# AmandineBtto/NeRAF

Hardware: AMD Instinct MI355X
Metric: field-samples/sec (rays + RIR STFT bins) (higher is better)
Workload: dtype f16; 1 GPU; RAF FurnishedRoom joint training step (BASELINE configs[2]): 4096 rays + 2048 RIR slices x 513 bins per GPU; radiance + grid refresh + ResNet3D + NAcF + STFT loss, backward, GradScaler + fused Adam...; rays_per_gpu=4096, slices_per_gpu=2048, global_rays=4096, global_slices=2048, parallelism=dp1, distinct_resident_batches=16, deterministic=True

## Files before the change

include/neraf_hip.h:

```cpp
#ifndef NERAF_HIP_H
#define NERAF_HIP_H

#include <stddef.h>
#include <stdint.h>

#ifdef __cplusplus
extern "C" {
#endif

typedef struct neraf_ctx neraf_ctx;
typedef void* neraf_stream_t;

enum {
  NERAF_OK = 0,
  NERAF_EINVAL = -1,
  NERAF_EHIP = -2,
  NERAF_ENOGPU = -3,
  NERAF_ESTATE = -4
};

#define NERAF_ABI_VERSION 1

int neraf_abi_version(void);
int neraf_ctx_create(neraf_ctx** out, int device);
void neraf_ctx_destroy(neraf_ctx* ctx);
const char* neraf_last_error(neraf_ctx* ctx);

int neraf_graph_stats(neraf_ctx* ctx, int* captures, int* launches);
int neraf_prof_enable(neraf_ctx* ctx, int on);
int neraf_prof_summary(neraf_ctx* ctx, int kernel_id, double* total_ms, int* launches, double* work);
int neraf_prof_summary_ex(neraf_ctx* ctx, int kernel_id, double* total_ms, int* launches, double* work, double* exec_work);
int neraf_prof_event_overhead(neraf_ctx* ctx, void* scratch_word, neraf_stream_t stream, double* ms);
const char* neraf_prof_kernel_name(int kernel_id);

int neraf_gemm_f16(neraf_ctx* ctx, const void* A, int lda, const void* B, int ldb, int M, int N, int K,
                   int Mpad, int Npad, float alpha, const float* bias, int act,
                   void* C16, int ldc16, void* C16T, int ldc16t, float* C32, int ldc32,
                   neraf_stream_t stream);

int neraf_gemm_f16_grouped(neraf_ctx* ctx, int ngroups, const void* const* A, const void* const* B, const int* M, const int* N,
                           float* const* C32, const int* ldc32, int lda, int ldb, int K, float alpha, const float* alpha_dev,
                           int c32_beta, void* splitk_ws, size_t splitk_bytes, neraf_stream_t stream);

int neraf_gemm_f16_stream(neraf_ctx* ctx, const void* A, int lda, const void* B, int ldb, int M, int N, int K, int Mpad, int Npad,
                          float alpha, const float* bias, const void* add16, int ldadd, void* C16, int ldc16, void* C16T,
                          int ldc16t, float* C32, int ldc32, float* colsum, float* colsumsq, int stat_rep, int stat_stride,
                          int stat_det, int body, int max_workgroups, neraf_stream_t stream);

int neraf_gemm_bf16(neraf_ctx* ctx, const void* A, int lda, const void* B, int ldb, int M, int N, int K,
                    int Mpad, int Npad, float alpha, const float* bias, int act,
                    void* C16, int ldc16, void* C16T, int ldc16t, float* C32, int ldc32,
                    neraf_stream_t stream);
int neraf_gemm_bf16_tn(neraf_ctx* ctx, const void* A, const void* B, int M, int N, int K, float* C32, void* splitk_ws,
                       size_t splitk_bytes, neraf_stream_t stream);

typedef struct neraf_nacf_desc {
  int n_feat;
  int n_query;
  int W;
  int C;
  int F;
  int dense_l0;
} neraf_nacf_desc;

size_t neraf_nacf_packed_bytes(const neraf_nacf_desc* d);
size_t neraf_nacf_workspace_bytes(const neraf_nacf_desc* d, int B, int training);

int neraf_nacf_pack_weights(neraf_ctx* ctx, const neraf_nacf_desc* d, const float* const* weights,
                            void* packed, neraf_stream_t stream);

int neraf_nacf_encode_queries(neraf_ctx* ctx, const neraf_nacf_desc* d, const int64_t* time_query,
                              const double* mic_pose, const double* source_pose, const double* rot,
                              const float* aabb_host, int max_len, int B, void* workspace, int training,
                              neraf_stream_t stream);
int neraf_nacf_encode_queries_ex(neraf_ctx* ctx, const neraf_nacf_desc* d, const int64_t* time_query,
                                 const double* mic_pose, const double* source_pose, const double* rot, int pose_rows,
                                 const float* aabb_host, int max_len, int B, void* workspace, int training,
                                 neraf_stream_t stream);

int neraf_nacf_fwd(neraf_ctx* ctx, const neraf_nacf_desc* d, const void* packed, const float* const* weights,
                   const float* feat, int B, float* out, void* workspace, int training, neraf_stream_t stream);

int neraf_nacf_fwd_dense(neraf_ctx* ctx, const neraf_nacf_desc* d, const void* packed, const float* h, int B,
                         float* out, void* workspace, int training, neraf_stream_t stream);

int neraf_nacf_bwd(neraf_ctx* ctx, const neraf_nacf_desc* d, const void* packed, const float* const* weights,
                   const float* feat, int B, const float* out, const float* dout, float* const* grads,
                   float* dfeat, void* workspace, neraf_stream_t stream);

int neraf_nacf_bwd_dense(neraf_ctx* ctx, const neraf_nacf_desc* d, const void* packed, int B, const float* out,
                         const float* dout, float* const* grads, float* dh, void* workspace,
                         neraf_stream_t stream);

#define NERAF_STFT_SUMS_FLOATS (4 + 4 * 256)
int neraf_stft_loss_fwd(neraf_ctx* ctx, const float* pred, const float* gt, size_t n, int loss_type,
                        float* sums, float* losses, neraf_stream_t stream);
int neraf_stft_loss_sums(neraf_ctx* ctx, const float* pred, const float* gt, size_t n, int loss_type,
                         float* sums, neraf_stream_t stream);
int neraf_stft_loss_finalize(neraf_ctx* ctx, const float* sums, size_t n_total, const float* weights, float* losses,
                             neraf_stream_t stream);
// ... 200 lines not shown
```

neraf_amd/_lib.py:

```python
from __future__ import annotations

import ctypes as C
import os
from typing import Dict, Optional

_HERE = os.path.dirname(os.path.abspath(__file__))
LIB_PATH = os.environ.get("NERAF_HIP_LIB") or os.path.join(_HERE, "libneraf_hip.so")

_lib: Optional[C.CDLL] = None
_ctxs: Dict[int, C.c_void_p] = {}

c_fpp = C.POINTER(C.c_void_p)


class GridDesc(C.Structure):
    _fields_ = [("n_levels", C.c_int), ("base_res", C.c_int), ("max_res", C.c_int), ("log2_hashmap_size", C.c_int),
                ("n_features", C.c_int)]


class ResnetDesc(C.Structure):
    _fields_ = [("grid_size", C.c_int), ("in_channels", C.c_int), ("n_features", C.c_int)]


class NacfDesc(C.Structure):
    _fields_ = [("n_feat", C.c_int), ("n_query", C.c_int), ("W", C.c_int), ("C", C.c_int), ("F", C.c_int),
                ("dense_l0", C.c_int)]


SIGNATURES = {
    "neraf_abi_version": (C.c_int, []),
    "neraf_ctx_create": (C.c_int, [C.POINTER(C.c_void_p), C.c_int]),
    "neraf_ctx_destroy": (None, [C.c_void_p]),
    "neraf_last_error": (C.c_char_p, [C.c_void_p]),
    "neraf_gemm_f16": (C.c_int, [C.c_void_p, C.c_void_p, C.c_int, C.c_void_p, C.c_int, C.c_int, C.c_int, C.c_int,
                                 C.c_int, C.c_int, C.c_float, C.c_void_p, C.c_int, C.c_void_p, C.c_int, C.c_void_p,
                                 C.c_int, C.c_void_p, C.c_int, C.c_void_p]),
    "neraf_gemm_f16_grouped": (C.c_int, [C.c_void_p, C.c_int, c_fpp, c_fpp, C.POINTER(C.c_int), C.POINTER(C.c_int), c_fpp,
                                         C.POINTER(C.c_int), C.c_int, C.c_int, C.c_int, C.c_float, C.c_void_p, C.c_int, C.c_void_p, C.c_size_t,
                                         C.c_void_p]),
    "neraf_gemm_f16_stream": (C.c_int, [C.c_void_p, C.c_void_p, C.c_int, C.c_void_p, C.c_int, C.c_int, C.c_int, C.c_int, C.c_int, C.c_int,
                                        C.c_float, C.c_void_p, C.c_void_p, C.c_int, C.c_void_p, C.c_int, C.c_void_p, C.c_int, C.c_void_p,
                                        C.c_int, C.c_void_p, C.c_void_p, C.c_int, C.c_int, C.c_int, C.c_int, C.c_int, C.c_void_p]),
    "neraf_gemm_bf16": (C.c_int, [C.c_void_p, C.c_void_p, C.c_int, C.c_void_p, C.c_int, C.c_int, C.c_int, C.c_int,
                                  C.c_int, C.c_int, C.c_float, C.c_void_p, C.c_int, C.c_void_p, C.c_int, C.c_void_p,
                                  C.c_int, C.c_void_p, C.c_int, C.c_void_p]),
    "neraf_gemm_bf16_tn": (C.c_int, [C.c_void_p, C.c_void_p, C.c_void_p, C.c_int, C.c_int, C.c_int, C.c_void_p, C.c_void_p, C.c_size_t,
                                     C.c_void_p]),
    "neraf_fused_adam_chunk": (C.c_int, []),
    "neraf_grads_nonfinite": (C.c_int, [C.c_void_p, C.c_void_p, C.c_void_p, C.c_void_p, C.c_void_p, C.c_int, C.c_void_p, C.c_void_p, C.c_int,
                                        C.c_int, C.c_void_p]),
    "neraf_fused_adam": (C.c_int, [C.c_void_p, C.c_void_p, C.c_void_p, C.c_void_p, C.c_void_p, C.c_int, C.c_void_p, C.c_int, C.c_int,
                                   C.c_double, C.c_double, C.c_double, C.c_void_p, C.c_void_p, C.c_void_p, C.c_void_p]),
    "neraf_fused_adam_dual": (C.c_int, [C.c_void_p, C.c_void_p, C.c_void_p, C.c_void_p, C.c_void_p, C.c_int, C.c_void_p, C.c_int, C.c_int,
                                        C.c_double, C.c_double, C.c_double, C.c_void_p, C.c_void_p, C.c_void_p, C.c_void_p, C.c_void_p,
                                        C.c_void_p, C.c_void_p, C.c_int, C.c_void_p, C.c_int, C.c_void_p]),
    "neraf_nacf_packed_bytes": (C.c_size_t, [C.POINTER(NacfDesc)]),
    "neraf_nacf_workspace_bytes": (C.c_size_t, [C.POINTER(NacfDesc), C.c_int, C.c_int]),
    "neraf_nacf_pack_weights": (C.c_int, [C.c_void_p, C.POINTER(NacfDesc), c_fpp, C.c_void_p, C.c_void_p]),
    "neraf_nacf_encode_queries": (C.c_int, [C.c_void_p, C.POINTER(NacfDesc), C.c_void_p, C.c_void_p, C.c_void_p,
                                            C.c_void_p, C.POINTER(C.c_float), C.c_int, C.c_int, C.c_void_p, C.c_int,
                                            C.c_void_p]),
    "neraf_nacf_encode_queries_ex": (C.c_int, [C.c_void_p, C.POINTER(NacfDesc), C.c_void_p, C.c_void_p, C.c_void_p,
                                               C.c_void_p, C.c_int, C.POINTER(C.c_float), C.c_int, C.c_int, C.c_void_p, C.c_int,
                                               C.c_void_p]),
    "neraf_nacf_fwd": (C.c_int, [C.c_void_p, C.POINTER(NacfDesc), C.c_void_p, c_fpp, C.c_void_p, C.c_int, C.c_void_p,
                                 C.c_void_p, C.c_int, C.c_void_p]),
    "neraf_nacf_fwd_dense": (C.c_int, [C.c_void_p, C.POINTER(NacfDesc), C.c_void_p, C.c_void_p, C.c_int, C.c_void_p,
                                       C.c_void_p, C.c_int, C.c_void_p]),
    "neraf_nacf_bwd": (C.c_int, [C.c_void_p, C.POINTER(NacfDesc), C.c_void_p, c_fpp, C.c_void_p, C.c_int, C.c_void_p,
                                 C.c_void_p, c_fpp, C.c_void_p, C.c_void_p, C.c_void_p]),
    "neraf_nacf_bwd_dense": (C.c_int, [C.c_void_p, C.POINTER(NacfDesc), C.c_void_p, C.c_int, C.c_void_p, C.c_void_p,
                                       c_fpp, C.c_void_p, C.c_void_p, C.c_void_p]),
    "neraf_stft_loss_fwd": (C.c_int, [C.c_void_p, C.c_void_p, C.c_void_p, C.c_size_t, C.c_int, C.c_void_p, C.c_void_p,
                                      C.c_void_p]),
    "neraf_stft_loss_sums": (C.c_int, [C.c_void_p, C.c_void_p, C.c_void_p, C.c_size_t, C.c_int, C.c_void_p, C.c_void_p]),
    "neraf_stft_loss_finalize": (C.c_int, [C.c_void_p, C.c_void_p, C.c_size_t, C.c_void_p, C.c_void_p, C.c_void_p]),
    "neraf_stft_loss_bwd": (C.c_int, [C.c_void_p, C.c_void_p, C.c_void_p, C.c_size_t, C.c_size_t, C.c_int, C.c_void_p,
                                      C.c_void_p, C.c_void_p, C.c_void_p, C.c_float, C.c_void_p, C.c_void_p]),
    "neraf_prof_event_overhead": (C.c_int, [C.c_void_p, C.c_void_p, C.c_void_p, C.POINTER(C.c_double)]),
    "neraf_graph_stats": (C.c_int, [C.c_void_p, C.POINTER(C.c_int), C.POINTER(C.c_int)]),
    "neraf_prof_enable": (C.c_int, [C.c_void_p, C.c_int]),
    "neraf_prof_summary": (C.c_int, [C.c_void_p, C.c_int, C.POINTER(C.c_double), C.POINTER(C.c_int), C.POINTER(C.c_double)]),
    "neraf_prof_summary_ex": (C.c_int, [C.c_void_p, C.c_int, C.POINTER(C.c_double), C.POINTER(C.c_int), C.POINTER(C.c_double),
                                        C.POINTER(C.c_double)]),
    "neraf_prof_kernel_name": (C.c_char_p, [C.c_int]),
    "neraf_grid_layout": (C.c_int, [C.POINTER(GridDesc), C.POINTER(C.c_float), C.POINTER(C.c_int), C.POINTER(C.c_uint32),
                                    C.POINTER(C.c_uint32)]),
    "neraf_hash_encode": (C.c_int, [C.c_void_p, C.POINTER(GridDesc), C.c_void_p, C.c_void_p, C.c_longlong, C.c_void_p, C.c_void_p]),
    "neraf_sample_uniform": (C.c_int, [C.c_void_p, C.c_int, C.c_int, C.c_float, C.c_float, C.c_void_p, C.c_uint64, C.c_void_p,
                                       C.c_void_p, C.c_void_p]),
    "neraf_proposal_density": (C.c_int, [C.c_void_p, C.POINTER(GridDesc), C.c_void_p, C.c_void_p, C.c_void_p, C.c_void_p,
                                         C.c_void_p, C.c_int, C.c_int, C.c_float, C.c_int, C.c_void_p, C.c_void_p]),
    "neraf_proposal_density_ex": (C.c_int, [C.c_void_p, C.POINTER(GridDesc), C.c_void_p, C.c_void_p, C.c_void_p, C.c_void_p,
                                            C.c_void_p, C.c_int64, C.c_int, C.c_int, C.c_float, C.c_int, C.c_void_p, C.c_void_p]),
    "neraf_pdf_resample_ex": (C.c_int, [C.c_void_p, C.c_void_p, C.c_void_p, C.c_void_p, C.c_int64, C.c_int, C.c_int, C.c_float,
# ... 163 lines not shown
```

neraf_amd/csrc/common.h:

```cpp
#pragma once
#include <hip/hip_runtime.h>
#include <stdint.h>
#include <stdio.h>
#include <new>
#include <string>
#include <vector>

#include "../../include/neraf_hip.h"

typedef _Float16 half_t;
typedef _Float16 half8 __attribute__((ext_vector_type(8)));
typedef _Float16 half4 __attribute__((ext_vector_type(4)));
typedef _Float16 half2v __attribute__((ext_vector_type(2)));
typedef __bf16 bf16_t;
typedef __bf16 bf16x8 __attribute__((ext_vector_type(8)));
typedef __bf16 bf16x4 __attribute__((ext_vector_type(4)));
typedef float f32x4 __attribute__((ext_vector_type(4)));
typedef float f32x16 __attribute__((ext_vector_type(16)));

enum { PROF_GEMM128 = 0, PROF_GEMM64 = 1, PROF_PROP_DENSITY = 2, PROF_FIELD_QUERY = 3, PROF_CONV = 4, PROF_PROP_BWD = 5, PROF_FIELD_BWD = 6,
       PROF_FIELD_SCATTER = 7, PROF_GEMM_WIDE = 8, PROF_WGRAD = 9, PROF_GEMM64_BF16 = 10, PROF_GEMM12864 = 11,
       PROF_CONV64_BF16 = 12, PROF_CONV12864 = 13, PROF_CONV128 = 14, PROF_CONV_STEM = 15, PROF_NUM_KERNELS = 16 };

struct ProfRec { hipEvent_t a, b; int kid; double work; double exec; };
// ... 124 lines not shown
  size_t blocks = (words + 256 - 1) / 256;
  if (blocks > 4096) blocks = 4096;
  hipLaunchKernelGGL(neraf_zero3_kernel, dim3((unsigned)blocks), dim3(256), 0, st, (unsigned*)p0, w0, (unsigned*)p1, w1, (unsigned*)p2, w2);
}

static inline bool neraf_deterministic() {
  static const bool d = [] { const char* e = getenv("NERAF_DETERMINISTIC"); return e && atoi(e) != 0; }();
  return d;
}

static inline int round_up(int x, int m) { return (x + m - 1) / m * m; }
static inline size_t round_up_sz(size_t x, size_t m) { return (x + m - 1) / m * m; }

enum { ACT_NONE = 0, ACT_LEAKY = 1, ACT_TANH10 = 2, ACT_RELU = 3 };

struct ConvGeom {
  int loader;
  int din, dout, stride, pad, ksize, cin;
  int tflip;
  int tstride;
  int tclass;
  const half_t* zero_page;
};

struct GemmParams {
  const half_t* A; int lda;
  const half_t* B; int ldb;
  int M, N, K;
  int Mpad, Npad;
  float alpha;
  const float* alpha_dev;
  const float* bias;
  int act;
  const half_t* lmask; int ldmask;
  float mask_slope;
  const half_t* add16; int ldadd;
  half_t* C16; int ldc16;
  half_t* C16T; int ldc16t;
  float* C32; int ldc32;
  int c32_beta;
  float* colsum;
  float* colsumsq;
  int stat_rep, stat_stride;
  int stat_det;
  const half_t* bnb_x; int ldbnb;
  const half_t* bnb_mask;
  const float* bnb_fin; int bnb_cpad;
  ConvGeom conv;
  float* splitk_ws; size_t splitk_ws_bytes;
  int tile_n;
  double alg_flops;
  int bf16;
  int stream_body, stream_max_wg;
  int ngroups;
  struct Group { const half_t* A; const half_t* B; float* C32; int M, N, ldc32; int tile_begin; } grp[6];
};
constexpr int kMaxGemmGroups = 6;

int launch_gemm_f16(neraf_ctx* ctx, const GemmParams& p, hipStream_t stream);

struct WgradItem {
  const void* dy;
  const void* x;
  float* out;
  int cout, cin, cin_real, ksize, stride, pad, din, dout;
  int K;
  int alpha_idx;
};
int launch_wgrad_grouped(neraf_ctx* ctx, const WgradItem* items, int n, const half_t* zero_page, float* slab_ws, size_t slab_bytes,
                         const float* alpha_dev, hipStream_t stream, bool bf16 = false);

constexpr int kAmaxRep = 32, kAmaxStride = 64;
```

neraf_amd/csrc/gemm_f16.hip:

```cpp
#include "common.h"
#include <stdlib.h>
#include <type_traits>

namespace {

constexpr int BK = 64;

__device__ __forceinline__ float act_apply(float v, int act) {
  if (act == ACT_LEAKY) return v > 0.f ? v : 0.1f * v;
  if (act == ACT_TANH10) return 10.f * tanhf(v);
  if (act == ACT_RELU) return v > 0.f ? v : 0.f;
  return v;
}

template <bool BF> struct ET;
template <> struct ET<false> {
  typedef _Float16 s; typedef half8 v8; typedef half4 v4;
  static __device__ __forceinline__ f32x4 mfma(v8 a, v8 b, f32x4 c) { return __builtin_amdgcn_mfma_f32_16x16x32_f16(a, b, c, 0, 0, 0); }
};
template <> struct ET<true> {
  typedef __bf16 s; typedef bf16x8 v8; typedef bf16x4 v4;
  static __device__ __forceinline__ f32x4 mfma(v8 a, v8 b, f32x4 c) { return __builtin_amdgcn_mfma_f32_16x16x32_bf16(a, b, c, 0, 0, 0); }
};

// ... 679 lines not shown
  __shared__ float tile2[32][33];
  if (p.bnb_x) {
#pragma unroll
    for (int r = 0; r < 4; ++r) tile2[row][c4 + r] = v[r] * (((float)xv[r] - mu[r]) * rsqrtf(var[r] + 1e-5f));
  }
  if (p.C16) {
    E4 h;
#pragma unroll
    for (int r = 0; r < 4; ++r) h[r] = (E)v[r];
    *reinterpret_cast<E4*>(reinterpret_cast<E*>(p.C16) + (size_t)m * p.ldc16 + n) = h;
  }
  if (C32 && m < M) {
    float* dst = C32 + (size_t)m * ldc32 + n;
    if (n + 3 < N && (reinterpret_cast<size_t>(dst) & 15) == 0) {
      f32x4 o = v;
      if (p.c32_beta) o += *reinterpret_cast<const f32x4*>(dst);
      *reinterpret_cast<f32x4*>(dst) = o;
    } else {
#pragma unroll
      for (int r = 0; r < 4; ++r) if (n + r < N) dst[r] = v[r] + (p.c32_beta ? dst[r] : 0.f);
    }
  }
  __syncthreads();
  const int tx = t & 31, ty = t >> 5;
  if (p.C16T) {
#pragma unroll
    for (int i = 0; i < 4; ++i) {
      const int nn = n0 + ty + i * 8, mm = m0 + tx;
      reinterpret_cast<E*>(p.C16T)[(size_t)nn * p.ldc16t + mm] = (E)tile[tx][ty + i * 8];
    }
  }
  if ((p.colsum || p.colsumsq) && ty < 2) {
    float cs = 0.f;
    if (ty == 0) {
#pragma unroll 8
      for (int i = 0; i < 32; ++i) cs += tile[i][tx];
    } else if (p.bnb_x) {
#pragma unroll 8
      for (int i = 0; i < 32; ++i) cs += tile2[i][tx];
    } else {
#pragma unroll 8
      for (int i = 0; i < 32; ++i) { const float x = tile[i][tx]; cs += x * x; }
    }
    float* dst = ty == 0 ? p.colsum : p.colsumsq;
    if (p.stat_det) {
      if (dst) dst[(size_t)blockIdx.y * p.stat_stride + n0 + tx] = cs;
    } else {
      const int rep = p.stat_rep > 1 ? (blockIdx.y & (p.stat_rep - 1)) * p.stat_stride : 0;
      if (dst) atomicAdd(dst + rep + n0 + tx, cs);
    }
  }
}

static void gemm_manifest(neraf_ctx* ctx, const GemmParams& p, int loader, int splits, int bm, int bn, double flops, bool wide = false, bool stream = false) {
  double out_elems = (double)p.M * p.N;
  double rA = loader == 0 ? (double)p.M * p.K * 2.0 : (double)p.conv.din * p.conv.din * p.conv.din * p.conv.cin * 2.0;
  double rB = (double)p.N * p.K * 2.0;
  const int ng = p.ngroups > 1 ? p.ngroups : 1;
  if (ng > 1) {
    out_elems = rA = rB = 0.0;
    for (int g = 0; g < ng; ++g) { out_elems += (double)p.grp[g].M * p.grp[g].N; rA += (double)p.grp[g].M * p.K * 2.0; rB += (double)p.grp[g].N * p.K * 2.0; }
  }
  const double epi_r = out_elems * 2.0 * ((p.add16 ? 1 : 0) + (p.lmask ? 1 : 0) + (p.bnb_mask ? 1 : 0) + (p.bnb_x ? 1 : 0));
  const double epi_w = out_elems * (2.0 * ((p.C16 ? 1 : 0) + (p.C16T ? 1 : 0)) + (p.C32 ? 4.0 : 0.0));
  const double slabs = (double)splits * ng * p.Mpad * p.Npad * 4.0;
  char nm[96];
  if (ng > 1)
    snprintf(nm, sizeof(nm), "gemm_f16_nt_pipe_kernel<%d, %d | plain, %d groups, %.0f results K=%d%s", bm, bn, ng, out_elems, p.K, splits > 1 ? " splitK" : "");
  else
    snprintf(nm, sizeof(nm), "%s<%d, %d | %s M=%d N=%d K=%d%s",
             stream ? "gemm_f16_nt_stream_kernel" : (wide ? "gemm_f16_nt_wide_kernel" : "gemm_f16_nt_pipe_kernel"), bm, bn,
             loader == 0 ? "plain" : (p.conv.tflip ? "dgrad" : "conv"), p.M, p.N, p.K, splits > 1 ? " splitK" : "");
  if (splits > 1) {
    neraf_node(ctx, nm, flops, rA + rB, slabs);
    neraf_node(ctx, "splitk_reduce_kernel | K-split slabs -> result", 0.0, slabs + epi_r, epi_w);
  } else {
    neraf_node(ctx, nm, flops, rA + rB + epi_r, epi_w);
  }
}

template <int BM, int BN, int NST, int LOADER, int KS, bool BF, bool TC = false, int NW = 4, bool GRP = false>
int launch_pipe(neraf_ctx* ctx, const GemmParams& p_in, int splits, hipStream_t stream) {
  using PT = PipeTile<BM, BN, NST>;
  GemmParams p = p_in;
  if ((p.ngroups > 1) != GRP) return neraf_fail(ctx, NERAF_EINVAL, "gemm: grouped launches take the grouped instantiation");
  int grp_tiles = 0;
  if (GRP) {
    for (int g = 0; g < p.ngroups; ++g) {
      p.grp[g].tile_begin = grp_tiles;
      grp_tiles += ((p.grp[g].M + BM - 1) / BM) * ((p.grp[g].N + BN - 1) / BN);
    }
  }
  static bool attr_set = false;
  if (!attr_set) {
    NERAF_HIP_CHECK(ctx, hipFuncSetAttribute(reinterpret_cast<const void*>(&gemm_f16_nt_pipe_kernel<BM, BN, NST, LOADER, KS, BF, TC, NW, GRP>),
                                             hipFuncAttributeMaxDynamicSharedMemorySize, PT::LDS_BYTES));
    attr_set = true;
  }
  const int ng = p.ngroups > 1 ? p.ngroups : 1;
  const int ntiles = GRP ? grp_tiles : (p.Mpad / BM) * (p.Npad / BN);
  double flops = 2.0 * p.M * p.N * p.K;
  if (ng > 1) { flops = 0.0; for (int g = 0; g < ng; ++g) flops += 2.0 * p.grp[g].M * p.grp[g].N * p.K; }
  const double exec_flops = (LOADER != 0 && p.conv.tstride > 1) ? (p.alg_flops > 0.0 ? p.alg_flops : flops) : flops;
  if (p.alg_flops > 0.0) flops = p.alg_flops;
  constexpr int kid = LOADER == 2 ? PROF_CONV_STEM
                      : LOADER == 1 ? (BM * BN == 128 * 128 ? PROF_CONV128 : (BM == 128 ? PROF_CONV12864 : (BF ? PROF_CONV64_BF16 : PROF_CONV)))
                                    : (BM * BN == 128 * 128 ? PROF_GEMM128 : (BM == 128 ? PROF_GEMM12864 : (BF ? PROF_GEMM64_BF16 : PROF_GEMM64)));
  ProfScope prof(ctx, stream, kid, flops, exec_flops);
  hipLaunchKernelGGL((gemm_f16_nt_pipe_kernel<BM, BN, NST, LOADER, KS, BF, TC, NW, GRP>), dim3(ntiles * splits), dim3(NW * 64), PT::LDS_BYTES,
                     stream, p, splits);
  NERAF_HIP_CHECK(ctx, hipGetLastError());
  if (ctx && ctx->manifest) gemm_manifest(ctx, p, LOADER, splits, BM, BN, flops);
  if (splits > 1) {
    hipLaunchKernelGGL(splitk_reduce_kernel<BF>, dim3(p.Npad / 32, p.Mpad / 32, ng), dim3(256), 0, stream, p, splits);
    NERAF_HIP_CHECK(ctx, hipGetLastError());
  }
  return NERAF_OK;
}


template <int BM, int BN, int NST, bool BF>
int launch_wide(neraf_ctx* ctx, const GemmParams& p, int splits, hipStream_t stream) {
  using T = Tile<BM, BN, 4>;
  constexpr int LDS_BYTES = (NST * T::STAGE_BYTES > T::NWAVES * T::EPI_BYTES_WAVE) ? NST * T::STAGE_BYTES : T::NWAVES * T::EPI_BYTES_WAVE;
// ... 154 lines not shown
          red[(wave * 2 + 1) * NW + col] = y;
        }
      }
    __syncthreads();
    if (tid < 2 * NW) {
      const int which = tid / NW, col = tid - which * NW;
      float v = 0.f;
#pragma unroll
      for (int w = 0; w < 8; ++w) v += red[(w * 2 + which) * NW + col];
      float* dst = which ? p.colsumsq : p.colsum;
      if (dst) {
        if (p.stat_det) dst[(size_t)((2 * rg * R) >> 5) * p.stat_stride + n_w0 + col] = v;
        else atomicAdd(dst + (p.stat_rep > 1 ? (rg & (p.stat_rep - 1)) * p.stat_stride : 0) + n_w0 + col, v);
      }
    }
  }
}

static bool stream_qualifies(const GemmParams& p) {
  const bool nk = (p.N == 64 || p.N == 128 || p.N == 256) && (p.K == 64 || p.K == 128 || p.K == 256) && p.N * p.K <= 16384;
  return nk && p.Npad == p.N && p.conv.loader == 0 && p.ngroups <= 1 && !p.bf16 && (p.Mpad % kStreamRows) == 0 && p.C16 &&
         !p.bias && !p.act && !p.lmask && !p.C16T && !p.C32 && !p.alpha_dev && !p.bnb_x && !p.bnb_mask &&
         (!p.add16 || (p.ldadd % 4) == 0);
}

template <int N, int K>
int launch_stream_nk(neraf_ctx* ctx, const GemmParams& p, hipStream_t stream) {
  const int nblocks = p.Mpad / kStreamRows;
  constexpr int CS = stream_slices(N);
  int nrg = (ctx ? ctx->num_cus : 256) / CS;
  if (p.stream_max_wg > 0 && nrg > p.stream_max_wg / CS) nrg = p.stream_max_wg / CS;
  if (nrg > (nblocks + 1) / 2) nrg = (nblocks + 1) / 2;
  if (nrg < 1) nrg = 1;
  const int grid = nrg * CS;
  const double flops = p.alg_flops > 0.0 ? p.alg_flops : 2.0 * p.M * p.N * p.K;
  ProfScope prof(ctx, stream, N == 64 ? PROF_GEMM12864 : PROF_GEMM_WIDE, flops, 2.0 * p.M * p.N * p.K);
  if (p.colsum || p.colsumsq) hipLaunchKernelGGL((gemm_f16_nt_stream_kernel<N, K, true>), dim3(grid), dim3(512), 0, stream, p, nblocks, nrg);
  else hipLaunchKernelGGL((gemm_f16_nt_stream_kernel<N, K, false>), dim3(grid), dim3(512), 0, stream, p, nblocks, nrg);
  NERAF_HIP_CHECK(ctx, hipGetLastError());
  if (ctx && ctx->manifest) gemm_manifest(ctx, p, 0, 1, N, K, flops, false, true);
  return NERAF_OK;
}

int launch_stream(neraf_ctx* ctx, const GemmParams& p, hipStream_t stream) {
  switch (p.N * 1000 + p.K) {
    case 64064: return launch_stream_nk<64, 64>(ctx, p, stream);
    case 64128: return launch_stream_nk<64, 128>(ctx, p, stream);
    case 64256: return launch_stream_nk<64, 256>(ctx, p, stream);
    case 128064: return launch_stream_nk<128, 64>(ctx, p, stream);
    case 128128: return launch_stream_nk<128, 128>(ctx, p, stream);
    case 256064: return launch_stream_nk<256, 64>(ctx, p, stream);
  }
  return neraf_fail(ctx, NERAF_EINVAL, "gemm: shape outside the streaming body's");
}

struct WgDesc {
  const void* dy; const void* x; float* out;
  unsigned long long slab_off;
  int block_begin; int K;
  unsigned short cout, cin, cin_real, taps, din, tiles_n, splits;
  unsigned char dl, stride, ksize, loader; signed char pad; unsigned char mh, ai, r2, r3, r4;
};
static_assert(sizeof(WgDesc) == 64, "descriptor table must fit the 4 KiB kernel-argument segment");
constexpr int kMaxWg = 56;
struct WgTable { int n; int total_blocks; const half_t* zero_page; const float* alpha_dev; float* slab; int order; WgDesc d[kMaxWg]; };

__device__ __forceinline__ int wg_find(const WgTable& t, int bid) {
  int lo = 0, hi = t.n - 1;
  while (lo < hi) { const int mid = (lo + hi + 1) >> 1; if (t.d[mid].block_begin <= bid) lo = mid; else hi = mid - 1; }
  return lo;
}

__device__ __forceinline__ size_t wg_out_index(const WgDesc& d, int m, int n) {
  const int tap = n / d.cin, c = n - tap * d.cin;
  return ((size_t)m * d.cin_real + c) * d.taps + tap;
}

template <bool BF> struct TrRead;
template <> struct TrRead<true> {
  static __device__ __forceinline__ bf16x4 rd(const char* p) {
    return __builtin_amdgcn_ds_read_tr16_b64_v4bf16((__attribute__((address_space(3))) bf16x4*)p);
  }
};
template <> struct TrRead<false> {
  typedef __fp16 fp16x4 __attribute__((ext_vector_type(4)));
  static __device__ __forceinline__ half4 rd(const char* p) {
    const fp16x4 v = __builtin_amdgcn_ds_read_tr16_b64_v4f16((__attribute__((address_space(3))) fp16x4*)p);
    return __builtin_bit_cast(half4, v);
  }
};

template <int NST, bool BF>
__global__ __launch_bounds__(256) void wgrad_grouped_tn_kernel(WgTable t) {
  using E = typename ET<BF>::s; using E4 = typename ET<BF>::v4; using E8 = typename ET<BF>::v8;
  constexpr int BM = 64, BN = 64;
  constexpr int STAGE_BYTES = (BM + BN) * 128;
  extern __shared__ __attribute__((aligned(16))) char smem[];
  const int tid = threadIdx.x;
  const int lane = tid & 63;
  const int wave = __builtin_amdgcn_readfirstlane(tid >> 6);
  const int wm = wave >> 1, wn = wave & 1;
  const int gi = wg_find(t, blockIdx.x);
  const WgDesc& D = t.d[gi];
  int bid = blockIdx.x - D.block_begin;
  const int splits = D.splits, tiles_n = D.tiles_n, tiles_m = D.cout / BM;
  const int split = bid % splits;
// ... 367 lines not shown
    *reinterpret_cast<f32x4*>(slab + (size_t)(m_base + row) * Npad + n_base + col) = v;
  }
}

struct WgRedTable { int n; const float* alpha_dev; const float* slab; int tile_begin[kMaxWg + 1]; unsigned char item[kMaxWg]; };

__device__ __forceinline__ int wg_red_cb(const WgDesc& D) { return D.taps == 1 ? (D.cin < 256 ? D.cin : 256) : (D.taps > 32 ? D.cin : (D.cin < 128 ? D.cin : 128)); }

__global__ __launch_bounds__(256) void wgrad_grouped_reduce_kernel(WgTable t, WgRedTable r) {
  __shared__ float blk[3584];
  int lo = 0, hi = r.n - 1;
  const int bid = blockIdx.x;
  while (lo < hi) { const int mid = (lo + hi + 1) >> 1; if (r.tile_begin[mid] <= bid) lo = mid; else hi = mid - 1; }
  const WgDesc& D = t.d[r.item[lo]];
  const int tile = bid - r.tile_begin[lo];
  const int taps = D.taps, cin = D.cin, CB = wg_red_cb(D), cbs = cin / CB;
  const int m = tile / cbs, ci0 = (tile - m * cbs) * CB;
  const int Npad = D.tiles_n * 64;
  const size_t slab = (size_t)D.cout * Npad;
  const float* src = r.slab + D.slab_off + (size_t)m * Npad + ci0;
  const int splits = D.splits, pitch = taps + 1, q4 = CB >> 2, total4 = q4 * taps;
  for (int e = threadIdx.x; e < total4; e += 256) {
    const int tap = e / q4, c = (e - tap * q4) * 4;
    const float* p = src + tap * cin + c;
    f32x4 v = f32x4{0.f, 0.f, 0.f, 0.f};
    int s2 = 0;
    for (; s2 + 8 <= splits; s2 += 8) {
      f32x4 a[8];
#pragma unroll
      for (int u = 0; u < 8; ++u) a[u] = *reinterpret_cast<const f32x4*>(p + (size_t)(s2 + u) * slab);
#pragma unroll
      for (int u = 0; u < 8; ++u) v += a[u];
    }
    for (; s2 < splits; ++s2) v += *reinterpret_cast<const f32x4*>(p + (size_t)s2 * slab);
#pragma unroll
    for (int k = 0; k < 4; ++k) blk[taps == 1 ? c + k : (c + k) * pitch + tap] = v[k];
  }
  __syncthreads();
  const float alpha = r.alpha_dev ? r.alpha_dev[D.ai] : 1.f;
  const int creal = (D.cin_real - ci0) < CB ? (D.cin_real - ci0) : CB;
  float* dst = D.out + ((size_t)m * D.cin_real + ci0) * taps;
  for (int j = threadIdx.x; j < creal * taps; j += 256) {
    const int c = j / taps, tap = j - c * taps;
    dst[j] = blk[taps == 1 ? c : c * pitch + tap] * alpha;
  }
}

static const int kWide = [] { const char* e = getenv("NERAF_GEMM_WIDE"); return e ? atoi(e) : 1; }();
static const int kSplitMinK = [] { const char* e = getenv("NERAF_SPLIT_MIN_K"); return e ? atoi(e) : 32; }();

static bool conv_waves8() { static const bool v = [] { const char* e = getenv("NERAF_CONV_WAVES"); return e && atoi(e) == 8; }(); return v; }

constexpr int kStreamMinM = 32768;

template <int LOADER, int KS, bool BF>
int dispatch_tile(neraf_ctx* ctx, const GemmParams& p_in, hipStream_t stream) {
  GemmParams p = p_in;
  const int cus = ctx ? ctx->num_cus : 256;
  static const int kTclass = [] { const char* e = getenv("NERAF_DGRAD_TCLASS"); return e ? atoi(e) : 1; }();
  p.conv.tclass = 0;
  if (LOADER == 1 && kTclass && p.conv.tstride == 2 && p.conv.tflip && (p.conv.dout & 1) == 0 && p.ngroups <= 1 &&
      p.Mpad == p.conv.dout * p.conv.dout * p.conv.dout && (p.Mpad % 512) == 0 && (p.Npad % 64) == 0 && !p.lmask && !p.C16T && !p.C32 &&
      !p.colsum && !p.colsumsq) {
    p.conv.tclass = 1;
    if constexpr (LOADER == 1) { if (conv_waves8()) return launch_pipe<64, 64, 4, LOADER, KS, BF, true, 8>(ctx, p, 1, stream); }
    return launch_pipe<64, 64, 4, LOADER, KS, BF, LOADER == 1>(ctx, p, 1, stream);
  }
  if (p.stream_body == 1 && !(LOADER == 0 && !BF && stream_qualifies(p)))
    return neraf_fail(ctx, NERAF_EINVAL, "gemm: shape or epilogue outside the streaming body's");
  if constexpr (LOADER == 0 && !BF) {
    const bool det_stats = p.stat_det && (p.colsum || p.colsumsq);
    if (p.stream_body != 2 && stream_qualifies(p) && (p.stream_body == 1 || (p.Mpad >= kStreamMinM && !det_stats)))
      return launch_stream(ctx, p, stream);
  }
  const int nk = p.K / BK;
  int bm = 128, bn = 128;
  const bool can128 = (p.Mpad % 128) == 0 && (p.Npad % 128) == 0;
  static const int kTile64 = [] { const char* e = getenv("NERAF_CONV_TILE64"); return e ? atoi(e) : 1; }();
  if (p.tile_n == 64 && (p.Mpad % 128) == 0 && !(kTile64 && LOADER == 1)) { bm = 128; bn = 64; }
  else if (!can128 || (p.Mpad / 128) * (p.Npad / 128) < cus) { bm = 64; bn = 64; }
  const int ng = p.ngroups > 1 ? p.ngroups : 1;
  int ntiles = (p.Mpad / bm) * (p.Npad / bn);
  bool uniform = true;
  if (ng > 1) {
    bm = 64; bn = 64; ntiles = 0;
    for (int g = 0; g < ng; ++g) {
      ntiles += (round_up(p.grp[g].M, 64) / 64) * (round_up(p.grp[g].N, 64) / 64);
      uniform = uniform && round_up(p.grp[g].M, 64) == p.Mpad && round_up(p.grp[g].N, 64) == p.Npad;
    }
  }
  int splits = 1;
  static const int kOversub = [] { const char* e = getenv("NERAF_SPLIT_OVERSUB"); const int v = e ? atoi(e) : 2; return v < 1 ? 1 : (v > 4 ? 4 : v); }();
  if (p.splitk_ws && uniform && ntiles * 2 <= cus && nk >= kSplitMinK) {
    splits = ((LOADER != 0 && ntiles >= 64) ? kOversub : 1) * cus / ntiles;
    if (splits > nk / 4) splits = nk / 4;
    if (splits > 128) splits = 128;
    while (splits >= 2 && (size_t)splits * ng * p.Mpad * p.Npad * 4 > p.splitk_ws_bytes) splits >>= 1;
    if (splits < 2) splits = 1;
  }
  if (LOADER == 0 && ng == 1 && kWide && (p.Mpad % 256) == 0) {
    if ((p.Npad % 160) == 0 && (p.Mpad / 256) * (p.Npad / 160) * 4 >= cus * 3) return launch_wide<256, 160, 3, BF>(ctx, p, 1, stream);
    if ((p.Npad % 128) == 0 && (p.Mpad / 256) * (p.Npad / 128) >= cus) return launch_wide<256, 128, 3, BF>(ctx, p, 1, stream);
  }
  if (LOADER == 0 && ng == 1 && kWide && bm == 128 && bn == 128 && splits == 1 && ntiles < 2 * cus)
    return launch_wide<128, 128, 3, BF>(ctx, p, 1, stream);
  static const int kTile32 = [] { const char* e = getenv("NERAF_TILE32"); return e ? atoi(e) : 128; }();
  if constexpr (LOADER == 0) {
    if (ng > 1) {
      if (kTile32 && splits == 1 && ntiles <= kTile32) return launch_pipe<32, 32, 4, LOADER, KS, BF, false, 4, true>(ctx, p, 1, stream);
      return launch_pipe<64, 64, 4, LOADER, KS, BF, false, 4, true>(ctx, p, splits, stream);
    }
    if (kTile32 && splits == 1 && bm == 64 && bn == 64 && ntiles <= kTile32 && !p.C16T)
      return launch_pipe<32, 32, 4, LOADER, KS, BF>(ctx, p, 1, stream);
  }
  if (bm == 128 && bn == 128) return launch_pipe<128, 128, 2, LOADER, KS, BF>(ctx, p, splits, stream);
  if (bm == 128 && bn == 64) return launch_pipe<128, 64, 3, LOADER, KS, BF>(ctx, p, splits, stream);
  if constexpr (LOADER == 1) { if (conv_waves8()) return launch_pipe<64, 64, 4, LOADER, KS, BF, false, 8>(ctx, p, splits, stream); }
  return launch_pipe<64, 64, 4, LOADER, KS, BF>(ctx, p, splits, stream);
}

}

int launch_wgrad_grouped(neraf_ctx* ctx, const WgradItem* items, int n, const half_t* zero_page, float* slab_ws, size_t slab_bytes,
                         const float* alpha_dev, hipStream_t stream, bool bf16) {
  if (n <= 0 || n > kMaxWg || !items || !zero_page) return neraf_fail(ctx, NERAF_EINVAL, "wgrad_grouped: bad arguments");
  static const int nst = [] { const char* e = getenv("NERAF_WGRAD_NST"); const int v = e ? atoi(e) : 3; return v < 2 ? 2 : (v > 4 ? 4 : v); }();
// ... 136 lines not shown
      if (p.conv.ksize == 1) return p.bf16 ? dispatch_tile<1, 1, true>(ctx, p, stream) : dispatch_tile<1, 1, false>(ctx, p, stream);
      return neraf_fail(ctx, NERAF_EINVAL, "conv loader 1: ksize must be 1 or 3");
    case 2:
      if (p.conv.cin != 8 || p.conv.ksize != 5 || !p.conv.zero_page || p.bf16) return neraf_fail(ctx, NERAF_EINVAL, "conv loader 2: cin 8, ksize 5, fp16");
      return dispatch_tile<2, 5, false>(ctx, p, stream);
  }
  return neraf_fail(ctx, NERAF_EINVAL, "gemm: unknown loader");
}

extern "C" int neraf_gemm_f16(neraf_ctx* ctx, const void* A, int lda, const void* B, int ldb, int M, int N, int K,
                              int Mpad, int Npad, float alpha, const float* bias, int act, void* C16, int ldc16,
                              void* C16T, int ldc16t, float* C32, int ldc32, neraf_stream_t stream) {
  GemmParams p{};
  p.A = (const half_t*)A; p.lda = lda; p.B = (const half_t*)B; p.ldb = ldb;
  p.M = M; p.N = N; p.K = K; p.Mpad = Mpad; p.Npad = Npad; p.alpha = alpha; p.bias = bias; p.act = act;
  p.C16 = (half_t*)C16; p.ldc16 = ldc16; p.C16T = (half_t*)C16T; p.ldc16t = ldc16t; p.C32 = C32; p.ldc32 = ldc32;
  return launch_gemm_f16(ctx, p, (hipStream_t)stream);
}

extern "C" int neraf_gemm_f16_grouped(neraf_ctx* ctx, int ngroups, const void* const* A, const void* const* B, const int* M, const int* N,
                                      float* const* C32, const int* ldc32, int lda, int ldb, int K, float alpha, const float* alpha_dev,
                                      int c32_beta, void* splitk_ws, size_t splitk_bytes, neraf_stream_t stream) {
  if (ngroups < 1 || ngroups > kMaxGemmGroups || !A || !B || !M || !N || !C32 || !ldc32)
    return neraf_fail(ctx, NERAF_EINVAL, "gemm_f16_grouped: 1 to 6 groups");
  GemmParams p{};
  p.lda = lda; p.ldb = ldb; p.K = K; p.alpha = alpha; p.alpha_dev = alpha_dev; p.c32_beta = c32_beta;
  p.splitk_ws = (float*)splitk_ws; p.splitk_ws_bytes = splitk_ws ? splitk_bytes : 0;
  for (int g = 0; g < ngroups; ++g) {
    if (M[g] <= 0 || N[g] <= 0) return neraf_fail(ctx, NERAF_EINVAL, "gemm_f16_grouped: M and N must be positive");
    GemmParams::Group& G = p.grp[g];
    G.A = (const half_t*)A[g]; G.B = (const half_t*)B[g]; G.C32 = C32[g]; G.M = M[g]; G.N = N[g]; G.ldc32 = ldc32[g];
    if (!G.A || !G.B || !G.C32) return neraf_fail(ctx, NERAF_EINVAL, "gemm_f16_grouped: null operand or result");
  }
  p.ngroups = ngroups;
  return launch_gemm_f16(ctx, p, (hipStream_t)stream);
}

extern "C" int neraf_gemm_f16_stream(neraf_ctx* ctx, const void* A, int lda, const void* B, int ldb, int M, int N, int K, int Mpad, int Npad,
                                     float alpha, const float* bias, const void* add16, int ldadd, void* C16, int ldc16, void* C16T,
                                     int ldc16t, float* C32, int ldc32, float* colsum, float* colsumsq, int stat_rep, int stat_stride,
                                     int stat_det, int body, int max_workgroups, neraf_stream_t stream) {
  if (body < 0 || body > 2 || max_workgroups < 0) return neraf_fail(ctx, NERAF_EINVAL, "gemm_f16_stream: body 0..2, max_workgroups >= 0");
  GemmParams p{};
  p.A = (const half_t*)A; p.lda = lda; p.B = (const half_t*)B; p.ldb = ldb;
  p.M = M; p.N = N; p.K = K; p.Mpad = Mpad; p.Npad = Npad; p.alpha = alpha; p.bias = bias;
  p.add16 = (const half_t*)add16; p.ldadd = ldadd;
  p.C16 = (half_t*)C16; p.ldc16 = ldc16; p.C16T = (half_t*)C16T; p.ldc16t = ldc16t; p.C32 = C32; p.ldc32 = ldc32;
  p.colsum = colsum; p.colsumsq = colsumsq; p.stat_rep = stat_rep; p.stat_stride = stat_stride; p.stat_det = stat_det;
  p.tile_n = N == 64 ? 64 : 0;
  p.stream_body = body; p.stream_max_wg = max_workgroups;
  return launch_gemm_f16(ctx, p, (hipStream_t)stream);
}

extern "C" int neraf_gemm_bf16(neraf_ctx* ctx, const void* A, int lda, const void* B, int ldb, int M, int N, int K,
                               int Mpad, int Npad, float alpha, const float* bias, int act, void* C16, int ldc16,
                               void* C16T, int ldc16t, float* C32, int ldc32, neraf_stream_t stream) {
  GemmParams p{};
  p.bf16 = 1;
  p.A = (const half_t*)A; p.lda = lda; p.B = (const half_t*)B; p.ldb = ldb;
  p.M = M; p.N = N; p.K = K; p.Mpad = Mpad; p.Npad = Npad; p.alpha = alpha; p.bias = bias; p.act = act;
  p.C16 = (half_t*)C16; p.ldc16 = ldc16; p.C16T = (half_t*)C16T; p.ldc16t = ldc16t; p.C32 = C32; p.ldc32 = ldc32;
  return launch_gemm_f16(ctx, p, (hipStream_t)stream);
}

extern "C" int neraf_gemm_bf16_tn(neraf_ctx* ctx, const void* A, const void* B, int M, int N, int K, float* C32, void* splitk_ws,
                                  size_t splitk_bytes, neraf_stream_t stream) {
  if (!A || !B || !C32 || M <= 0 || N <= 0 || K <= 0 || (M % 64) || (N % 64) || (K % 64) || !splitk_ws || splitk_bytes < 256)
    return neraf_fail(ctx, NERAF_EINVAL, "gemm_bf16_tn: M, N, K multiples of 64; scratch required");
  WgradItem it{};
  it.dy = A; it.x = B; it.out = C32;
  it.cout = M; it.cin = N; it.cin_real = N; it.ksize = 1; it.stride = 1; it.pad = 0; it.din = 1; it.dout = 1; it.K = K;
  return launch_wgrad_grouped(ctx, &it, 1, (const half_t*)splitk_ws, (float*)((char*)splitk_ws + 256), splitk_bytes - 256, nullptr,
                              (hipStream_t)stream, true);
}
```

Baseline: 268.5 million field-samples/s.

## Add LDS-resident halo kernel for 3x3x3 64-channel conv3d and its dgrad

```diff
diff --git a/include/neraf_hip.h b/include/neraf_hip.h
--- a/include/neraf_hip.h
+++ b/include/neraf_hip.h
@@ -46,6 +46,10 @@
                           float alpha, const float* bias, const void* add16, int ldadd, void* C16, int ldc16, void* C16T,
                           int ldc16t, float* C32, int ldc32, float* colsum, float* colsumsq, int stat_rep, int stat_stride,
                           int stat_det, int body, int max_workgroups, neraf_stream_t stream);
+
+int neraf_conv3d_f16_body(neraf_ctx* ctx, const void* x, const void* w, const void* zero_page, int edge_in, int edge_out, int cin,
+                          int cout, int ksize, int stride, int pad, int transposed, float alpha, void* C16, float* colsum,
+                          float* colsumsq, int stat_rep, int stat_stride, int stat_det, int body, neraf_stream_t stream);
 
 int neraf_gemm_bf16(neraf_ctx* ctx, const void* A, int lda, const void* B, int ldb, int M, int N, int K,
                     int Mpad, int Npad, float alpha, const float* bias, int act,
diff --git a/neraf_amd/_lib.py b/neraf_amd/_lib.py
--- a/neraf_amd/_lib.py
+++ b/neraf_amd/_lib.py
@@ -41,6 +41,9 @@
     "neraf_gemm_f16_stream": (C.c_int, [C.c_void_p, C.c_void_p, C.c_int, C.c_void_p, C.c_int, C.c_int, C.c_int, C.c_int, C.c_int, C.c_int,
                                         C.c_float, C.c_void_p, C.c_void_p, C.c_int, C.c_void_p, C.c_int, C.c_void_p, C.c_int, C.c_void_p,
                                         C.c_int, C.c_void_p, C.c_void_p, C.c_int, C.c_int, C.c_int, C.c_int, C.c_int, C.c_void_p]),
+    "neraf_conv3d_f16_body": (C.c_int, [C.c_void_p, C.c_void_p, C.c_void_p, C.c_void_p, C.c_int, C.c_int, C.c_int, C.c_int, C.c_int, C.c_int,
+                                        C.c_int, C.c_int, C.c_float, C.c_void_p, C.c_void_p, C.c_void_p, C.c_int, C.c_int, C.c_int, C.c_int,
+                                        C.c_void_p]),
     "neraf_gemm_bf16": (C.c_int, [C.c_void_p, C.c_void_p, C.c_int, C.c_void_p, C.c_int, C.c_int, C.c_int, C.c_int,
                                   C.c_int, C.c_int, C.c_float, C.c_void_p, C.c_int, C.c_void_p, C.c_int, C.c_void_p,
                                   C.c_int, C.c_void_p, C.c_int, C.c_void_p]),
diff --git a/neraf_amd/csrc/common.h b/neraf_amd/csrc/common.h
--- a/neraf_amd/csrc/common.h
+++ b/neraf_amd/csrc/common.h
@@ -200,6 +200,7 @@
   double alg_flops;
   int bf16;
   int stream_body, stream_max_wg;
+  int conv_body;
   int ngroups;
   struct Group { const half_t* A; const half_t* B; float* C32; int M, N, ldc32; int tile_begin; } grp[6];
 };
diff --git a/neraf_amd/csrc/gemm_f16.hip b/neraf_amd/csrc/gemm_f16.hip
--- a/neraf_amd/csrc/gemm_f16.hip
+++ b/neraf_amd/csrc/gemm_f16.hip
@@ -755,7 +755,8 @@
   }
 }
 
-static void gemm_manifest(neraf_ctx* ctx, const GemmParams& p, int loader, int splits, int bm, int bn, double flops, bool wide = false, bool stream = false) {
+static void gemm_manifest(neraf_ctx* ctx, const GemmParams& p, int loader, int splits, int bm, int bn, double flops, bool wide = false, bool stream = false,
+                          bool resident = false) {
   double out_elems = (double)p.M * p.N;
   double rA = loader == 0 ? (double)p.M * p.K * 2.0 : (double)p.conv.din * p.conv.din * p.conv.din * p.conv.cin * 2.0;
   double rB = (double)p.N * p.K * 2.0;
@@ -772,7 +773,7 @@
     snprintf(nm, sizeof(nm), "gemm_f16_nt_pipe_kernel<%d, %d | plain, %d groups, %.0f results K=%d%s", bm, bn, ng, out_elems, p.K, splits > 1 ? " splitK" : "");
   else
     snprintf(nm, sizeof(nm), "%s<%d, %d | %s M=%d N=%d K=%d%s",
-             stream ? "gemm_f16_nt_stream_kernel" : (wide ? "gemm_f16_nt_wide_kernel" : "gemm_f16_nt_pipe_kernel"), bm, bn,
+             resident ? "conv3_f16_resident_kernel" : stream ? "gemm_f16_nt_stream_kernel" : (wide ? "gemm_f16_nt_wide_kernel" : "gemm_f16_nt_pipe_kernel"), bm, bn,
              loader == 0 ? "plain" : (p.conv.tflip ? "dgrad" : "conv"), p.M, p.N, p.K, splits > 1 ? " splitK" : "");
   if (splits > 1) {
     neraf_node(ctx, nm, flops, rA + rB, slabs);
@@ -1033,6 +1034,161 @@
     case 256064: return launch_stream_nk<256, 64>(ctx, p, stream);
   }
   return neraf_fail(ctx, NERAF_EINVAL, "gemm: shape outside the streaming body's");
+}
+
+constexpr int kResHX = 10, kResHY = 6, kResHZ = 6, kResHalo = kResHX * kResHY * kResHZ;
+constexpr int kResImgLd = 64 + 8;
+static_assert(kResHalo % 8 == 0, "whole LDS-DMA wave-instructions of eight voxels");
+
+template <int FLIP, int STATS>
+__global__ __launch_bounds__(256) void conv3_f16_resident_kernel(GemmParams p) {
+  constexpr int KB = 54;
+  __shared__ __attribute__((aligned(16))) char halo[kResHalo * 128];
+  __shared__ __attribute__((aligned(16))) char img[128 * kResImgLd * 2];
+  typedef __attribute__((address_space(3))) void* lds_ptr_t;
+  typedef const __attribute__((address_space(1))) void* gbl_ptr_t;
+
+  const int tid = threadIdx.x;
+  const int lane = tid & 63;
+  const int wave = __builtin_amdgcn_readfirstlane(tid >> 6);
+  const int frow = lane & 15, fq = lane >> 4;
+  const int d = p.conv.dout;
+  int bid = blockIdx.x;
+  {
+    const int nblocks = (int)gridDim.x, q = nblocks >> 3, r = nblocks & 7;
+    const int xcd = bid & 7, idx = bid >> 3;
+    bid = (xcd < r ? xcd * (q + 1) : r * (q + 1) + (xcd - r) * q) + idx;
+  }
+  const int nbx = d >> 3, nby = d >> 2;
+  const int x0 = (bid % nbx) * 8, y0 = ((bid / nbx) % nby) * 4, z0 = (bid / (nbx * nby)) * 4;
+
+#pragma unroll
+  for (int it = 0; it < (kResHalo / 8 + 3) / 4; ++it) {
+    const int q = it * 4 + wave;
+    if (q < kResHalo / 8) {
+      const int v = q * 8 + (lane >> 3);
+      const int hx = v % kResHX, hy = (v / kResHX) % kResHY, hz = v / (kResHX * kResHY);
+      const int gx = x0 - 1 + hx, gy = y0 - 1 + hy, gz = z0 - 1 + hz;
+      const bool ok = (unsigned)gx < (unsigned)d && (unsigned)gy < (unsigned)d && (unsigned)gz < (unsigned)d;
+      const int c = (lane & 7) ^ (hx & 7);
+      const half_t* src = ok ? p.A + ((size_t)((gz * d + gy) * d + gx) * 64 + c * 8) : p.conv.zero_page;
+      __builtin_amdgcn_global_load_lds((gbl_ptr_t)src, (lds_ptr_t)(halo + q * 1024), 16, 0, 0);
+    }
+  }
+  constexpr int WPD = 8;
+  const half_t* wsrc = p.B + (size_t)(wave * 16 + (lane >> 2)) * p.ldb + (lane & 3) * 8;
+  half8 w[KB];
+  {
+#pragma unroll
+    for (int kb = 0; kb < WPD; ++kb) w[kb] = *reinterpret_cast<const half8*>(wsrc + kb * 32);
+  }
+  const int from = (frow * 4 + fq) * 4;
+  auto place = [&](half8& f) {
+    const uint4 raw = __builtin_bit_cast(uint4, f);
+    uint4 t;
+    t.x = (unsigned)__builtin_amdgcn_ds_bpermute(from, (int)raw.x);
+    t.y = (unsigned)__builtin_amdgcn_ds_bpermute(from, (int)raw.y);
+    t.z = (unsigned)__builtin_amdgcn_ds_bpermute(from, (int)raw.z);
+    t.w = (unsigned)__builtin_amdgcn_ds_bpermute(from, (int)raw.w);
+    f = __builtin_bit_cast(half8, t);
+  };
+  const int rx = frow & 7, ryl = frow >> 3;
+  int abase[3][2];
+#pragma unroll
+  for (int o = 0; o < 3; ++o)
+#pragma unroll
+    for (int ks = 0; ks < 2; ++ks) abase[o][ks] = (ryl * kResHX + rx) * 128 + (((ks * 4 + fq) ^ ((rx + o) & 7)) * 16);
+
+  f32x4 acc[8];
+#pragma unroll
+  for (int i = 0; i < 8; ++i) acc[i] = f32x4{0.f, 0.f, 0.f, 0.f};
+
+  wait_vmcnt<WPD>();
+  __syncthreads();
+
+  half8 xa[2][8];
+  auto read_block = [&](int kb, half8 (&x)[8]) {
+    const int tap = kb >> 1, ks = kb & 1;
+    const int tz = tap / 9, ty = (tap / 3) % 3, tx = tap % 3;
+    const int oz = FLIP ? 2 - tz : tz, oy = FLIP ? 2 - ty : ty, ox = FLIP ? 2 - tx : tx;
+#pragma unroll
+    for (int i = 0; i < 8; ++i)
+      x[i] = *reinterpret_cast<const half8*>(halo + abase[ox][ks] + ((((i >> 1) + oz) * kResHY + (2 * (i & 1) + oy)) * kResHX + ox) * 128);
+  };
+  read_block(0, xa[0]);
+  place(w[0]);
+  place(w[1]);
+  __builtin_amdgcn_sched_barrier(0);
+#pragma unroll
+  for (int kb = 0; kb < KB; ++kb) {
+    if (kb + 1 < KB) read_block(kb + 1, xa[(kb + 1) & 1]);
+    if (kb + WPD < KB) w[kb + WPD] = *reinterpret_cast<const half8*>(wsrc + (kb + WPD) * 32);
+    if (kb + 2 < KB) place(w[kb + 2]);
+#pragma unroll
+    for (int i = 0; i < 8; ++i)
+      acc[i] = __builtin_amdgcn_mfma_f32_16x16x32_f16(w[kb], xa[kb & 1][i], acc[i], 0, 0, 0);
+    __builtin_amdgcn_sched_barrier(0);
+  }
+
+  const float alpha = p.alpha;
+  half_t* im = reinterpret_cast<half_t*>(img);
+  f32x4 s = f32x4{0.f, 0.f, 0.f, 0.f}, s2 = s;
+#pragma unroll
+  for (int i = 0; i < 8; ++i) {
+    const f32x4 v = acc[i] * alpha;
+    if constexpr (STATS) { s += v; s2 += v * v; }
+    half4 h;
+#pragma unroll
+    for (int r = 0; r < 4; ++r) h[r] = (half_t)v[r];
+    *reinterpret_cast<half4*>(im + (i * 16 + frow) * kResImgLd + wave * 16 + fq * 4) = h;
+  }
+  __syncthreads();
+#pragma unroll
+  for (int it = 0; it < 4; ++it) {
+    const int idx = it * 256 + tid, row = idx >> 3, ch = idx & 7;
+    const uint4 dv = *reinterpret_cast<const uint4*>(im + row * kResImgLd + ch * 8);
+    const int m = ((z0 + (row >> 5)) * d + y0 + ((row >> 3) & 3)) * d + x0 + (row & 7);
+    *reinterpret_cast<uint4*>(p.C16 + (size_t)m * p.ldc16 + ch * 8) = dv;
+  }
+  if constexpr (STATS) {
+    const int rep = p.stat_rep > 1 ? (bid & (p.stat_rep - 1)) * p.stat_stride : 0;
+#pragma unroll
+    for (int r = 0; r < 4; ++r) {
+      const float x = row16_sum(s[r]), y = row16_sum(s2[r]);
+      if (frow == 0) {
+        const int col = wave * 16 + fq * 4 + r;
+        if (p.colsum) atomicAdd(p.colsum + rep + col, x);
+        if (p.colsumsq) atomicAdd(p.colsumsq + rep + col, y);
+      }
+    }
+  }
+}
+
+static bool resident_qualifies(const GemmParams& p) {
+  const ConvGeom& g = p.conv;
+  const long vox = (long)g.dout * g.dout * g.dout;
+  return g.loader == 1 && g.ksize == 3 && g.stride == 1 && g.tstride <= 1 && g.cin == 64 && p.N == 64 && p.Npad == 64 && p.K == 27 * 64 &&
+         g.din == g.dout && g.dout > 0 && (g.dout % 8) == 0 && g.pad == (g.tflip ? -1 : 1) && (long)p.M == vox && p.Mpad == p.M &&
+         g.zero_page && p.ngroups <= 1 && !p.bf16 && p.C16 && !p.bias && !p.act && !p.lmask && !p.add16 && !p.C16T && !p.C32 &&
+         !p.alpha_dev && !p.bnb_x && !p.bnb_mask && !(p.stat_det && (p.colsum || p.colsumsq));
+}
+
+int launch_resident(neraf_ctx* ctx, const GemmParams& p, hipStream_t stream) {
+  const int d = p.conv.dout;
+  const int grid = (d / 8) * (d / 4) * (d / 4);
+  const double flops = p.alg_flops > 0.0 ? p.alg_flops : 2.0 * p.M * p.N * p.K;
+  const bool stats = p.colsum || p.colsumsq;
+  ProfScope prof(ctx, stream, PROF_CONV, flops, 2.0 * p.M * p.N * p.K);
+  if (p.conv.tflip) {
+    if (stats) hipLaunchKernelGGL((conv3_f16_resident_kernel<1, 1>), dim3(grid), dim3(256), 0, stream, p);
+    else hipLaunchKernelGGL((conv3_f16_resident_kernel<1, 0>), dim3(grid), dim3(256), 0, stream, p);
+  } else {
+    if (stats) hipLaunchKernelGGL((conv3_f16_resident_kernel<0, 1>), dim3(grid), dim3(256), 0, stream, p);
+    else hipLaunchKernelGGL((conv3_f16_resident_kernel<0, 0>), dim3(grid), dim3(256), 0, stream, p);
+  }
+  NERAF_HIP_CHECK(ctx, hipGetLastError());
+  if (ctx && ctx->manifest) gemm_manifest(ctx, p, 1, 1, p.conv.tflip ? 1 : 0, stats ? 1 : 0, flops, false, false, true);
+  return NERAF_OK;
 }
 
 struct WgDesc {
@@ -1506,6 +1662,7 @@
 static bool conv_waves8() { static const bool v = [] { const char* e = getenv("NERAF_CONV_WAVES"); return e && atoi(e) == 8; }(); return v; }
 
 constexpr int kStreamMinM = 32768;
+constexpr int kResidentMinM = 32768;
 
 template <int LOADER, int KS, bool BF>
 int dispatch_tile(neraf_ctx* ctx, const GemmParams& p_in, hipStream_t stream) {
@@ -1526,6 +1683,11 @@
     const bool det_stats = p.stat_det && (p.colsum || p.colsumsq);
     if (p.stream_body != 2 && stream_qualifies(p) && (p.stream_body == 1 || (p.Mpad >= kStreamMinM && !det_stats)))
       return launch_stream(ctx, p, stream);
+  }
+  if (p.conv_body == 1 && !(LOADER == 1 && KS == 3 && !BF && resident_qualifies(p)))
+    return neraf_fail(ctx, NERAF_EINVAL, "gemm: convolution or epilogue outside the resident body's");
+  if constexpr (LOADER == 1 && KS == 3 && !BF) {
+    if (p.conv_body != 2 && resident_qualifies(p) && (p.conv_body == 1 || p.Mpad >= kResidentMinM)) return launch_resident(ctx, p, stream);
   }
   const int nk = p.K / BK;
   int bm = 128, bn = 128;
@@ -1768,6 +1930,28 @@
   return launch_gemm_f16(ctx, p, (hipStream_t)stream);
 }
 
+extern "C" int neraf_conv3d_f16_body(neraf_ctx* ctx, const void* x, const void* w, const void* zero_page, int edge_in, int edge_out, int cin,
+                                     int cout, int ksize, int stride, int pad, int transposed, float alpha, void* C16, float* colsum,
+                                     float* colsumsq, int stat_rep, int stat_stride, int stat_det, int body, neraf_stream_t stream) {
+  if (body < 0 || body > 2 || !x || !w || !zero_page || !C16 || edge_in <= 0 || edge_out <= 0 || edge_out > 512 || cin <= 0 || cout <= 0 ||
+      ksize <= 0 || stride <= 0)
+    return neraf_fail(ctx, NERAF_EINVAL, "conv3d_f16_body: body 0..2, operands and positive extents");
+  GemmParams p{};
+  const int taps = ksize * ksize * ksize;
+  p.A = (const half_t*)x; p.lda = cin;
+  p.K = round_up(taps * cin, 64);
+  p.B = (const half_t*)w; p.ldb = p.K;
+  p.M = edge_out * edge_out * edge_out; p.N = cout; p.Mpad = round_up(p.M, 128); p.Npad = round_up(cout, 64);
+  p.alpha = alpha; p.C16 = (half_t*)C16; p.ldc16 = cout; p.tile_n = cout == 64 ? 64 : 0;
+  p.colsum = colsum; p.colsumsq = colsumsq; p.stat_rep = stat_rep; p.stat_stride = stat_stride; p.stat_det = stat_det;
+  p.conv.loader = cin == 8 ? 2 : 1; p.conv.din = edge_in; p.conv.dout = edge_out; p.conv.ksize = ksize; p.conv.cin = cin;
+  p.conv.zero_page = (const half_t*)zero_page;
+  if (transposed) { p.conv.stride = 1; p.conv.pad = -pad; p.conv.tflip = 1; p.conv.tstride = stride; }
+  else { p.conv.stride = stride; p.conv.pad = pad; }
+  p.conv_body = body;
+  return launch_gemm_f16(ctx, p, (hipStream_t)stream);
+}
+
 extern "C" int neraf_gemm_bf16(neraf_ctx* ctx, const void* A, int lda, const void* B, int ldb, int M, int N, int K,
                                int Mpad, int Npad, float alpha, const float* bias, int act, void* C16, int ldc16,
                                void* C16T, int ldc16t, float* C32, int ldc32, neraf_stream_t stream) {
```

Result: faster. 271.4 million field-samples/s, median of 6 (+1.1%).
